# microsoft/PDP-Solver

Measured on AMD Instinct MI355X. Metric: pdp_iterations_per_sec, higher is better.
Workload: dtype f32; 1 GPU; configs[1]: 'p-d-p' survey propagation, random 3-SAT n=200 m=840 batch=5000 T=100 per GPU; E=12600000, V=999999, F=4200000, algorithmic_bytes_per_launch=19540000000, semantics=reference (batch-wide couplings reproduced), parallelism=instances sharded, dp1

## Files before the change

### pdp-solver_amd/csrc/pdp_solve.hip

```cpp
#include "pdp_device.hpp"
#include <stdlib.h>
#include <algorithm>
#include <vector>
#include <type_traits>

#define ST(s) ((hipStream_t)(s))
#define PDP_RETRY_WITH_FORCE (-77)

template <class IT>
struct SView {
    int b, n, m, e;
    const IT *e_var, *e_fn, *v_ptr, *v_edges, *f_ptr, *f_edges;
    const int8_t *sgn;
    float *av, *af, *sol;
    float *emask;
    float *qu; int qstride;
    float *eta; int estride;
    const float *force; int fstride;
    float *s0, *s1, *s2, *s3;
    float *S;
    float *P, *N, *xv1, *xv2, *score, *coeff, *assign;
    int32_t *deg, *sdeg;
    uint8_t *flag_v, *flag_f, *flag_f2;
};
// ... 40 lines not shown
    uint32_t *w_perm_zero, *w_iters_run, *w_violation;
    int team_size, team_count, team_slots;
    int team_no_xcd;
    int exact;
    int rf;
    int isolate;
    uint32_t *risk;
    int no_scorer_reuse;
    int no_event_look;
    int rf_no_fused_step;
    int debug_ghost_inject;
    int adopt_poison;
    int lds_tickets;
    uint8_t *ghost_flag;
    uint32_t *team_ws;
};

struct SolveCtl {
    uint32_t nan_iter;
    uint32_t perm_zero;
    uint32_t violation;
    uint32_t iters_run;
    uint32_t replay_count;
    uint32_t do_replay;
    int32_t poison_from;
    uint32_t ticket;
};
struct SolveCall {
    uint32_t poisoned_all;
    uint32_t stop;
// ... 964 lines not shown
            neg = neg + (negative ? 1.0f : 0.0f) * f;
            all = all + f;
        }
        const float sc = d_score_from_sums(pos, neg, all, ext, pi);
        if (check_score && sc != sc) bad = 1;
    }
    if (bad) cs->found = 1;
    __syncthreads();
    return cs->found;
}

#define DEC_FIXED 1
#define DEC_SPEC_SHIFT 1
#define DEC_VERIFIED_SHIFT 3
template <bool FORCE>
__device__ __noinline__ int lds_decimate(uint32_t smem_off, uint32_t cold_off, int nt, int n, int m, int ne, int cur, int active, float pi, int verified, int scorer_src)
{
    unsigned char *const smem = lds_at<unsigned char>(smem_off);
    ColdShared *const cs = lds_at<ColdShared>(cold_off);
    const LdsArrays L = carve_all(smem, n, m, ne);
    constexpr int VMD = FORCE ? PV_VMASK_RF : 0x3fff;
    const int tid = threadIdx.x, lane = tid & 63;
    float *Enew = cur ? L.EA : L.EB;
    float *score = L.xv2, *assign = L.coeff;
    DEC_PROF_DECL
    float *const SL = (scorer_src == 2) ? L.QU : L.Y;
    const int y_has_logs = scorer_src == 1;
    if (!y_has_logs) {
        const int full = ne / (4 * nt), rem = ne - full * 4 * nt, quarter = (rem + 3) >> 2;
        for (int k = 0; k <= full; ++k) {
            const bool tail = k == full;
// ... 4 lines not shown
            for (int j = 0; j < 4; ++j) { p[j] = p0 + j * st; in[j] = p[j] < ne; if (!in[j]) p[j] = p0; }
            const f4v lg = log4_fin((f4v){1.0f - Enew[p[0]], 1.0f - Enew[p[1]], 1.0f - Enew[p[2]], 1.0f - Enew[p[3]]}, PDP_SCORER_EPS);
            const float r[4] = {lg.x, lg.y, lg.z, lg.w};
#pragma unroll
            for (int j = 0; j < 4; ++j) if (in[j]) SL[p[j]] = r[j] * (0.0f + L.af[L.pcc[p[j]] & 0x3fff]);
        }
    }
    if (tid == 0) { cs->key = 0ull; cs->flags = 0; cs->found = 0; }
    __syncthreads();
    DEC_PROF_MARK(16);
    const float Lpi = pdp_safe_log(1.0f - pi, PDP_SCORER_EPS), L0 = pdp_safe_log(1.0f - pi * 0.0f, PDP_SCORER_EPS);
    const float clamp_sp = y_has_logs ? log2_fin((f2v){0.0f, 0.0f}, PDP_SP_EPS).x : __builtin_nanf(""), clamp_sc = log4_fin((f4v)(0.0f), PDP_SCORER_EPS).x;
    int flags = 0;
    unsigned long long key = 0ull;
    for (int i = tid; i < n; i += nt) {
        const int v = L.vord[i];
        float ext = 0.0f, pos = 0.0f, neg = 0.0f, all = 0.0f;
        auto acc = [&](float f, uint16_t pw, float frc) {
            const bool ng = (pw & 0x8000) != 0;
            f = (f == clamp_sp) ? clamp_sc : f;
            ext = ext + frc;
            pos = pos + (ng ? 0.0f : 1.0f) * f;
            neg = neg + (ng ? 1.0f : 0.0f) * f;
            all = all + f;
        };
        int p = L.v_ptr[v];
        const int bnd = L.v_ptr[v + 1];
        for (; p + 7 < bnd; p += 8) {
            float f[8], fr[8]; uint16_t pw[8];
#pragma unroll
            for (int j = 0; j < 8; ++j) { f[j] = SL[p + j]; pw[j] = L.pvv[p + j]; fr[j] = FORCE ? frc_of(pw[j]) : 0.0f; }
// ... 3 lines not shown
        for (; p + 3 < bnd; p += 4) {
            float f[4], fr[4]; uint16_t pw[4];
#pragma unroll
            for (int j = 0; j < 4; ++j) { f[j] = SL[p + j]; pw[j] = L.pvv[p + j]; fr[j] = FORCE ? frc_of(pw[j]) : 0.0f; }
#pragma unroll
            for (int j = 0; j < 4; ++j) acc(f[j], pw[j], fr[j]);
        }
        for (; p < bnd; ++p) { const uint16_t pw1 = L.pvv[p]; acc(SL[p], pw1, FORCE ? frc_of(pw1) : 0.0f); }
        const float sc = lds_score_of(pos, neg, all, ext, Lpi, L0);
        const float co = (pdp_abs(sc) * L.av[v]) * 1.0f;
        score[v] = sc; L.coeff[v] = co;
        L.flag_v[v] = 0;
        if (co == 0.0f) flags |= 1;
        if (co != 0.0f) flags |= 2;
        if (co != co) flags |= 4;
        const unsigned long long kv = argkey((co - 0.0f) + 1.0f, v);
        key = kv > key ? kv : key;
    }
    flags = wave_reduce(flags, OpOrI(), 0);
    key = wave_max_u64(key);
    if (lane == 63) { if (flags) atomicOr(&cs->flags, flags); if (key) atomicMax(&cs->key, key); }
    __syncthreads();
    flags = UNI(cs->flags);
    const int z3 = flags & 1, anynz = (flags >> 1) & 1, cn = (flags >> 2) & 1;
    int ret = ((z3 ? 1 : 0) | (cn ? 2 : 0)) << DEC_SPEC_SHIFT;
    DEC_PROF_MARK(17);
    const unsigned long long kwin = cs->key;
    const int li = UNI(argkey_index(kwin));
    if (!(active && anynz && !cn && li >= 0)) return ret | (verified << DEC_VERIFIED_SHIFT);
    const float sgn_li = pdp_sign(score[li]);
    DEC_PROF_MARK(18);
    const LView I = make_lview(L, 0, n, m, ne, nt, cs->red, VMD);
    SimplifyScratch ss;
    ss.assign = assign; ss.deg = reinterpret_cast<int32_t *>(L.xv1); ss.sdeg = reinterpret_cast<int32_t *>(L.xv2);
    ss.flag_v = L.flag_v; ss.flag_f = reinterpret_cast<uint8_t *>(L.S); ss.flag_f2 = ss.flag_f + ((m + 15) & ~15); ss.red = cs->red;

    if (verified == 0) {
        int bad = 0;
        for (int c = tid; c < m; c += nt) {
            if (L.af[c] == 1.0f) {
                float deg = 0.0f;
                for (int k = L.f_ptr[c]; k < L.f_ptr[c + 1]; ++k) deg = deg + L.av[L.pvv[L.e2p[k]] & VMD];
                if (deg == 1.0f) bad = 1;
// ... 71 lines not shown
#endif
        if (found & 1) d_simplify(I, ss, &cs->is_sat);
        else if (found & 2) d_peel(I, ss);
        return ret;
    }

    for (int v = tid; v < n; v += nt) assign[v] = 0.0f;
    __syncthreads();
    if (tid == 0) assign[li] = sgn_li;
    __syncthreads();
    d_set_variable_core(I, ss);
    d_simplify(I, ss, &cs->is_sat);
    return ret;
}

__device__ __noinline__ int lds_reinforce_step(uint32_t smem_off, uint32_t cold_off, int nt, int n, int m, int ne, int cur, float pi, int do_force, int logs)
{
    ColdShared *const cs = lds_at<ColdShared>(cold_off);
    const LdsArrays L = carve_all(lds_at<unsigned char>(smem_off), n, m, ne);
    const int tid = threadIdx.x;
    int bad = 0;
    const float *const Enew = cur ? L.EA : L.EB;
    float *const SL = (logs == 2) ? L.QU : L.Y;
    if (do_force && logs != 1) {
        for (int p = tid; p < ne; p += nt)
            SL[p] = pdp_safe_log_fin(1.0f - Enew[p], PDP_SCORER_EPS) * (0.0f + L.af[L.pcc[p] & 0x3fff]);
        __syncthreads();
    }
    const float clamp_sp = (logs == 1) ? pdp_safe_log_fin(0.0f, PDP_SP_EPS) : __builtin_nanf(""), clamp_sc = pdp_safe_log_fin(0.0f, PDP_SCORER_EPS);
    const float Lpi = pdp_safe_log(1.0f - pi, PDP_SCORER_EPS), L0 = pdp_safe_log(1.0f - pi * 0.0f, PDP_SCORER_EPS);
    uint32_t *const codev = reinterpret_cast<uint32_t *>(L.xv2);
    for (int i = tid; i < n; i += nt) {
        const int v = L.vord[i];
        const int a = L.v_ptr[v], bnd = L.v_ptr[v + 1];
        float pred;
        if (do_force) {
            float ext = 0.0f, pos = 0.0f, neg = 0.0f, all = 0.0f;
            const bool in_place = logs == 1 && L.av[v] == 1.0f;
            for (int p = a; p < bnd; ++p) {
                float f = SL[p];
                if (logs == 1) f = in_place ? ((f == clamp_sp) ? clamp_sc : f) : pdp_safe_log_fin(1.0f - Enew[p], PDP_SCORER_EPS) * (0.0f + L.af[L.pcc[p] & 0x3fff]);
                const uint16_t pw = L.pvv[p];
                const bool ng = (pw & 0x8000) != 0;
                ext = ext + frc_of(pw);
                pos = pos + (ng ? 0.0f : 1.0f) * f;
                neg = neg + (ng ? 1.0f : 0.0f) * f;
                all = all + f;
            }
// ... 90 lines not shown
            for (int p = tid; p < ne; p += nt) pvv[p] = (uint16_t)(spv[p] | (frc_enc(sp.frc_in[G.e0 + p]) << PV_FRC_SHIFT));
        }
        asm volatile("s_waitcnt vmcnt(0)" ::: "memory");
    }
    __shared__ __attribute__((aligned(16))) ColdShared s_cold;
    constexpr int SPEC_LOCAL = 64;
    __shared__ uint8_t s_spec_used[SPEC_LOCAL], s_spec_zero[SPEC_LOCAL];
    __shared__ int s_flag_or[2];
    __shared__ int s_sat_count;
    __shared__ uint32_t s_risk;
    __shared__ int s_poison;
    if (tid < SPEC_LOCAL) { s_spec_used[tid] = 0; s_spec_zero[tid] = 0; }
    if (tid == 0) { s_cold.is_sat = hdr.is_sat; s_flag_or[0] = 0; s_flag_or[1] = 0; s_sat_count = 0; s_risk = 0xffffffffu; }
    __syncthreads();

    const bool p4_cached = 2 * n <= nt;
    uint32_t p4_lohi = 0u, p4_vdeg = 0u;
    if (p4_cached && tid < 2 * n) {
        const int v = L.vord[tid >> 1], h = tid & 1;
        const int a = L.v_ptr[v], bnd = L.v_ptr[v + 1];
        const int half = (bnd - a + 1) >> 1;
        p4_lohi = (uint32_t)(a + h * half) | ((uint32_t)(h ? bnd : a + half) << 16);
        p4_vdeg = (uint32_t)v | ((uint32_t)(bnd - a) << 16);
    }
    int active = hdr.active ? 1 : 0;
    int has_prev = sp.has_prev;
    int last_event = -1;
    int prev_from_global = (sp.has_prev && sp.prev_slots) ? 1 : 0;
    int use_em = sp.has_edge_mask, last_use_em = 0, em_dirty = 0;
    float cnt = hdr.cnt;
    int iters = 0, did_prop = 0, violation = 0, cur = 0;
    int logs_ready = 0;
    int qu_is_delta = 0;
    int mask_fix = 0;
// ... 51 lines not shown
                if (((c >> 1) ^ c) & PC_EM_USED) pcc[p] = (uint16_t)((c & ~PC_EM_USED) | ((c & PC_EM) ? PC_EM_USED : 0));
            }
            __syncthreads();
            PROF_MARK(19);
        }
        last_use_em = use_em; em_dirty = 0; mask_fix = 0;
        PROF_MARK(1);
        {
            const uint16_t *const e2p = L.e2p, *const f_ptr = L.f_ptr, *const v_ptr = L.v_ptr;
            float *const S = L.S;
            const int nvi = (n + 63) >> 6, nci = (m + 63) >> 6;
            const uint16_t *const vord = L.vord;
            auto var_rows = [&](int item) {
                const int i = (item << 6) + lane;
                if (i >= n) return;
                const int v = vord[i];
                float P = 0.0f, N = 0.0f;
                const int a = v_ptr[v], bnd = v_ptr[v + 1];
                auto acc = [&](float y, uint16_t sg) {
                    const uint32_t neg = (uint32_t)((int32_t)((uint32_t)sg << 16) >> 31);
                    P = P + __uint_as_float(__float_as_uint(y) & ~neg);
                    N = N + __uint_as_float(__float_as_uint(y) & neg);
                };
                int p = a;
                for (; p + 15 < bnd; p += 16) {
                    float y[16]; uint16_t sg[16];
#pragma unroll
                    for (int j = 0; j < 16; ++j) { y[j] = Y[p + j]; sg[j] = pvv[p + j]; }
#pragma unroll
                    for (int j = 0; j < 16; ++j) acc(y[j], sg[j]);
                }
// ... 153 lines not shown
        qu_is_delta = logs_ready;
        float *const Dsrc = fuse_logs ? QU : Y;
        __syncthreads();
        PROF_MARK(3);
        int bits = nan_seen ? 4 : 0;
        {
            const uint16_t *const v_ptr = L.v_ptr;
            const float *const av = L.av;
            float *const amb = L.xv1;
            const float tol_lo = tol - (2e-6f + 1e-4f * pdp_abs(tol)), tol_hi = tol + (2e-6f + 1e-4f * pdp_abs(tol));
            if (!PROF_SKIP(8))
            for (int r = tid; r < 2 * n; r += nt) {
                int v, lo, hi, degi;
                if (p4_cached) { lo = (int)(p4_lohi & 0xffffu); hi = (int)(p4_lohi >> 16); v = (int)(p4_vdeg & 0xffffu); degi = (int)(p4_vdeg >> 16); }
                else {
                    v = L.vord[r >> 1];
                    const int h = r & 1, a = v_ptr[v], bnd = v_ptr[v + 1];
                    const int half = (bnd - a + 1) >> 1;
                    lo = a + h * half; hi = h ? bnd : a + half; degi = bnd - a;
                }
                float emax = 0.0f, S1 = 0.0f, S2 = 0.0f, D = 0.0f;
                if (has_prev) {
                    int p = lo;
                    for (; p + 1 < hi; p += 2) {
                        const float e0 = Enew[p], e1 = Enew[p + 1], d0 = Dsrc[p], d1 = Dsrc[p + 1];
                        emax = fmaxf(emax, fmaxf(e0, e1));
                        S1 += d0 + d1; S2 = fmaf(d0, d0, fmaf(d1, d1, S2)); D = fmaxf(D, fmaxf(d0, d1));
                    }
                    if (p < hi) { const float e0 = Enew[p], d0 = Dsrc[p]; emax = fmaxf(emax, e0); S1 += d0; S2 = fmaf(d0, d0, S2); D = fmaxf(D, d0); }
                } else {
                    for (int p = lo; p < hi; ++p) emax = fmaxf(emax, Enew[p]);
// ... 104 lines not shown
                conv = below_tol ? 1 : 0;
                if (cnt >= t_max) { conv = 1; cnt = 0.0f; }
                if (conv) last_event = t;
            }
        } else if (has_prev) {
            if (cnt >= t_max) { conv = 1; cnt = 0.0f; }
        }
        uint32_t used = (RF ? 0u : 1u) | (has_prev ? 2u : 0u);
        uint32_t zero = ((!RF && z1) ? 1u : 0u) | ((has_prev && z2) ? 2u : 0u);
        if (!RF && has_prev && !conv && n > 0) zero |= 4u;
        if constexpr (RF) {
            const int flip = (sp.coins[sp.chunk_start + t] < sp.dprob) && active;
            rf_last_flip = flip;
            if (flip || nsat < 0) {
                const int keep_logs = fuse_logs ? (use_em ? 1 : 2) : 0;
                if (UNI(lds_reinforce_step(lds_offset_of(smem), lds_offset_of(&s_cold), nt, n, m, ne, cur, pi, flip, keep_logs)) && !nan_seen) violation = 1;
                rf_changed = 1;
                if (!keep_logs) logs_ready = 0;
            }
        }
        PROF_MARK(13);
        int decimated = 0;
        if (!RF && has_prev && conv && !poisoned && !nan_seen && !PROF_SKIP(16)) {
            const int scorer_src = !fuse_logs ? 0 : ((use_em && !sp.no_scorer_reuse) ? 1 : 2);
            const int dr = UNI(lds_decimate<FORCE>(lds_offset_of(smem), lds_offset_of(&s_cold), nt, n, m, ne, cur, active, pi, simplified, scorer_src));
            decimated = dr & DEC_FIXED; simplified = (dr >> DEC_VERIFIED_SHIFT) & 3;
            const int spec_bits = (dr >> DEC_SPEC_SHIFT) & 3;
            used |= 4u;
            if (spec_bits & 1) zero |= 4u;
            if (spec_bits & 2) violation = 1;
        }
        if (decimated) { if (simplified == 1) PROF_COUNT(10); else PROF_COUNT(11); }
        PROF_COUNT(12);
        PROF_MARK(6);
        if (has_prev) cnt = cnt + 1.0f;
        if (tid == 0 && !poisoned) {
            if (t < SPEC_LOCAL) { s_spec_used[t] = (uint8_t)used; s_spec_zero[t] = (uint8_t)zero; }
            else { atomicOr(&sp.spec_used[t], used); if (zero) atomicOr(&sp.spec_zero[t], zero); }
        }
        {
// ... 50 lines not shown
            if (sp.check_termination && active && nsat == m) active = 0;
        }
        has_prev = 1; prev_from_global = 0; cur ^= 1;
        PROF_MARK(15);
    }

    int any_inactive = 0;
    for (int v = tid; v < n; v += nt) any_inactive |= (L.av[v] == 0.0f) ? 1 : 0;
    any_inactive = __syncthreads_or(any_inactive);
    const bool finishing = did_prop && (sp.final_chunk || !active);
    float *const Efin = cur ? L.EB : L.EA, *const Eprev = cur ? L.EA : L.EB;
    const bool ghost = finishing && !active && !(sp.final_chunk && iters >= T) && !sp.isolate;
    if (finishing) {
        float *gq = sp.q + 3 * (size_t)G.e0;
        float *gfs = sp.fs + 2 * (size_t)G.e0;
        for (int p = tid; p < ne; p += nt) {
            const int e = G.v_edges[p];
            const uint16_t pw = pvv[p], cw = pcc[p];
            const int v = pw & VM;
            const float s = slot_sign(pw);
            float y = pdp_safe_log_fin(1.0f - Eprev[p], PDP_SP_EPS);
            if (last_use_em) y = y * ((cw & PC_EM_USED) ? 1.0f : 0.0f);
            const float force = RF ? (rf_last_flip ? (qu_is_delta ? QU[p] : X[p]) : frc_of(pw)) : (FORCE ? frc_of(pw) : 0.0f);
            const float pos = 0.0f + L.PN[2 * v], neg = 0.0f + L.PN[2 * v + 1];
            float same = (0.5f * (1.0f + s)) * pos + (0.5f * (1.0f - s)) * neg;
            same = same - y;
            same = same + ((force == s) ? L1 : L0);
            float opp = (0.5f * (1.0f - s)) * pos + (0.5f * (1.0f + s)) * neg;
            opp = opp + ((force == -s) ? L1 : L0);
            const float dc = pdp_expf_fin_le30(same + opp);
            const float A = pdp_expf_fin_le30(same), Bv = pdp_expf_fin_le30(opp);
            const float qu = A * (1.0f - Bv), qs = Bv * (1.0f - A);
            const float total = (qu + qs) + dc;
            const float sticky = qu_is_delta ? __builtin_fmaf(1.0f - 1.0f, X[p], qu / total) : QU[p];
            const float sticky_out = (ghost && sp.debug_ghost_inject && p == 0) ? __builtin_nanf("") : sticky;
            if (ghost) QU[p] = sticky_out;
            gq[3 * e] = sticky_out;
            gq[3 * e + 1] = 1.0f * (qs / total) + (1.0f - 1.0f) * sticky;
            gq[3 * e + 2] = 1.0f * (dc / total) + (1.0f - 1.0f) * sticky;
            gfs[2 * e] = Efin[p];
            if constexpr (RF) gfs[2 * e + 1] = frc_of(pw);
            sp.prev[G.e0 + e] = Efin[p];
            G.emask[e] = (cw & PC_EM) ? 1.0f : 0.0f;
        }
        for (int v = tid; v < n; v += nt) { G.av[v] = L.av[v]; G.sol[v] = L.sol[v]; }
        for (int c = tid; c < m; c += nt) G.af[c] = L.af[c];
    } else {
        auto dump16 = [&](size_t off, const void *src, size_t bytes) {
            uint4 *g = reinterpret_cast<uint4 *>(dout + off);
            const uint4 *d = reinterpret_cast<const uint4 *>(src);
            for (int i = tid; i < (int)((bytes + 15) >> 4); i += nt) g[i] = d[i];
        };
        dump16(BL.QU, QU, (size_t)ne * 4); dump16(BL.E, Efin, (size_t)ne * 4);
        dump16(BL.af, L.af, (size_t)m * 4); dump16(BL.av, L.av, (size_t)n * 4); dump16(BL.sol, L.sol, (size_t)n * 4);
        uint16_t *gpc = reinterpret_cast<uint16_t *>(dout + BL.pcc);
        for (int p = tid; p < ne; p += nt) { const uint16_t cw = pcc[p]; gpc[p] = (uint16_t)((cw & ~PC_EM_USED) | ((cw & PC_EM) ? PC_EM_USED : 0)); }
        if constexpr (RF) { for (int p = tid; p < ne; p += nt) sp.frc_out[G.e0 + p] = frc_of(pvv[p]); }
    }
    int ghost_bad = 0;
    if (ghost) {
// ... 19 lines not shown
        if (!REPLAY) sp.last_event[gb] = last_event;
        if (sp.risk) sp.risk[gb] = finishing ? 0xffffffffu : s_risk;
        atomicMax(&ctl->iters_run, (uint32_t)iters);
        if (violation) atomicOr(&ctl->violation, 1u);
    }
}

struct SolveSnapshot {
    float *q, *fs, *av, *af, *sol, *sat, *emask, *prev, *cnt; uint8_t *amask;
};
__global__ void __launch_bounds__(256) k_solve_import(PView pv, const float *q, const float *fs, const uint8_t *amask, const float *prev, const float *counters,
                                                      int has_prev, int build_static, char *stat, char *dyn, const int64_t *stat_off, const int64_t *dyn_off, float *prev_slots,
                                                      const int32_t *list, int stage_cap ,
                                                      SolveCall *force_check ,
                                                      int use_em ,
                                                      SolveSnapshot snap )
{
    const Inst G = load_inst(pv, list ? list[blockIdx.x] : (int)blockIdx.x);
    const int n = G.n, m = G.m, ne = G.e, tid = threadIdx.x, nt = blockDim.x;
    const BlobLayout BL = blob_layout(n, m, ne);
    char *st = stat + stat_off[G.b], *dy = dyn + dyn_off[G.b];
    uint16_t *pvv = reinterpret_cast<uint16_t *>(st + BL.pvv), *e2p = reinterpret_cast<uint16_t *>(st + BL.e2p);
    float *QU = reinterpret_cast<float *>(dy + BL.QU), *Ecur = reinterpret_cast<float *>(dy + BL.E);
    uint16_t *pcc = reinterpret_cast<uint16_t *>(dy + BL.pcc);
    const float *sq = q + 3 * (size_t)G.e0, *sfs = fs + 2 * (size_t)G.e0;
    extern __shared__ __attribute__((aligned(16))) float stage[];
    if (force_check) {
        int some = 0;
        for (int e0 = tid; e0 < ne; e0 += 4 * nt) {
            float f[4];
#pragma unroll
            for (int j = 0; j < 4; ++j) { const int e = e0 + j * nt; f[j] = sfs[2 * (e < ne ? e : e0) + 1]; }
#pragma unroll
            for (int j = 0; j < 4; ++j) some |= (f[j] != 0.0f) ? 1 : 0;
        }
        if (__syncthreads_or(some) && tid == 0) atomicOr(&force_check->force_seen, 1u);
    }
// ... 7 lines not shown
                const int e = (e0 + j * nt < ne) ? e0 + j * nt : e0;
                qv[j] = sq[3 * e]; ev[j] = sfs[2 * e]; fn[j] = G.e_fn[e];
                if (use_em) mv[j] = G.emask[e];
                if (has_prev) pv[j] = prev[G.e0 + e];
            }
#pragma unroll
            for (int j = 0; j < 4; ++j) {
                const int e = e0 + j * nt;
                if (e >= ne) continue;
                sQ[e] = qv[j]; sE[e] = ev[j]; sC[e] = (uint16_t)(fn[j] | ((mv[j] == 1.0f) ? (PC_EM | PC_EM_USED) : 0));
                if (has_prev) sP[e] = pv[j];
            }
        }
        __syncthreads();
        for (int p0 = tid; p0 < ne; p0 += 8 * nt) {
            int e[8], evar[8], esg[8];
#pragma unroll
            for (int j = 0; j < 8; ++j) { const int p = p0 + j * nt; e[j] = G.v_edges[p < ne ? p : p0]; }
            if (build_static) {
#pragma unroll
                for (int j = 0; j < 8; ++j) { evar[j] = G.e_var[e[j]]; esg[j] = G.sgn[e[j]]; }
            }
#pragma unroll
            for (int j = 0; j < 8; ++j) {
                const int p = p0 + j * nt;
                if (p >= ne) continue;
                if (build_static) { pvv[p] = (uint16_t)(evar[j] | (esg[j] < 0 ? 0x8000 : 0)); e2p[e[j]] = (uint16_t)p; }
                pcc[p] = sC[e[j]];
                QU[p] = sQ[e[j]]; Ecur[p] = sE[e[j]];
                if (has_prev) prev_slots[G.e0 + p] = sP[e[j]];
            }
        }
    } else
    for (int p0 = tid; p0 < ne; p0 += 4 * nt) {
        int e[4]; float qv[4], ev[4], mv[4], pv[4] = {0.0f, 0.0f, 0.0f, 0.0f}; int fn[4];
#pragma unroll
        for (int j = 0; j < 4; ++j) { const int p = p0 + j * nt; e[j] = G.v_edges[p < ne ? p : p0]; }
#pragma unroll
        for (int j = 0; j < 4; ++j) {
            qv[j] = sq[3 * e[j]]; ev[j] = sfs[2 * e[j]]; mv[j] = use_em ? G.emask[e[j]] : 1.0f; fn[j] = G.e_fn[e[j]];
            if (has_prev) pv[j] = prev[G.e0 + e[j]];
        }
#pragma unroll
        for (int j = 0; j < 4; ++j) {
            const int p = p0 + j * nt;
            if (p >= ne) continue;
            if (build_static) { pvv[p] = (uint16_t)(G.e_var[e[j]] | (G.sgn[e[j]] < 0 ? 0x8000 : 0)); e2p[e[j]] = (uint16_t)p; }
            pcc[p] = (uint16_t)(fn[j] | ((mv[j] == 1.0f) ? (PC_EM | PC_EM_USED) : 0));
            QU[p] = qv[j]; Ecur[p] = ev[j];
            if (has_prev) prev_slots[G.e0 + p] = pv[j];
        }
    }
    if (build_static) {
        uint16_t *vp = reinterpret_cast<uint16_t *>(st + BL.vptr), *fp = reinterpret_cast<uint16_t *>(st + BL.fptr);
        for (int v = tid; v <= n; v += nt) vp[v] = (uint16_t)G.v_ptr[v];
        for (int c = tid; c <= m; c += nt) fp[c] = (uint16_t)G.f_ptr[c];
        __shared__ int hist[256];
        uint16_t *vord = reinterpret_cast<uint16_t *>(st + BL.vord);
        for (int i = tid; i < 256; i += nt) hist[i] = 0;
        __syncthreads();
        for (int v = tid; v < n; v += nt) { const int d = G.v_ptr[v + 1] - G.v_ptr[v]; atomicAdd(&hist[255 - (d < 255 ? d : 255)], 1); }
        __syncthreads();
        if (tid == 0) { int run = 0; for (int i = 0; i < 256; ++i) { const int c = hist[i]; hist[i] = run; run += c; } }
        __syncthreads();
        for (int v = tid; v < n; v += nt) { const int d = G.v_ptr[v + 1] - G.v_ptr[v]; vord[atomicAdd(&hist[255 - (d < 255 ? d : 255)], 1)] = (uint16_t)v; }
    }
    float *av = reinterpret_cast<float *>(dy + BL.av), *sol = reinterpret_cast<float *>(dy + BL.sol), *af = reinterpret_cast<float *>(dy + BL.af);
    int any_inactive = 0;
    for (int v = tid; v < n; v += nt) {
        const float a = G.av[v], so = G.sol[v];
        av[v] = a; sol[v] = so; any_inactive |= (a == 0.0f) ? 1 : 0;
        if (snap.av) { snap.av[G.v0 + v] = a; snap.sol[G.v0 + v] = so; }
    }
    for (int c = tid; c < m; c += nt) { const float f = G.af[c]; af[c] = f; if (snap.av) snap.af[G.f0 + c] = f; }
    any_inactive = __syncthreads_or(any_inactive);
    if (tid == 0) {
        if (snap.av) { snap.sat[G.b] = pv.is_sat[G.b]; snap.cnt[G.b] = counters[G.b]; snap.amask[G.b] = amask[G.b]; }
        DynHeader h;
        h.active = amask[G.b] ? 1u : 0u; h.done = h.active ? 0u : 1u;
        h.perm_zero = (h.done && any_inactive) ? 1u : 0u; h.simplified = 0;
        h.cnt = counters[G.b]; h.is_sat = pv.is_sat[G.b]; h.nsat_p1 = 0; h.pad2 = 0.0f;
        *reinterpret_cast<DynHeader *>(dy + BL.hdr) = h;
    }
}

__global__ void __launch_bounds__(256) k_force_import(PView pv, const float *fs, float *frc, SolveCtl *ctl0, const uint8_t *amask)
{
    const Inst G = load_inst(pv, blockIdx.x);
    if (!amask[G.b]) return;
    const float *sfs = fs + 2 * (size_t)G.e0;
    int odd = 0;
    for (int p = threadIdx.x; p < G.e; p += blockDim.x) {
        const float f = sfs[2 * G.v_edges[p] + 1];
        frc[G.e0 + p] = f;
        odd |= (f == f && f != 0.0f && f != 1.0f && f != -1.0f) ? 1 : 0;
    }
    if (__syncthreads_or(odd) && threadIdx.x == 0) atomicOr(&ctl0->violation, 1u);
}

__global__ void __launch_bounds__(1024) k_solve_post(SolveCtl *ctl, SolveCall *call, int c, int isolate, int B, const int32_t *last_event, int32_t *list,
                                                     const uint8_t *is_big)
{
    __shared__ int s_from;
    if (threadIdx.x == 0) {
        int from = -1;
        if (!call->stop) {
            ctl->do_replay = 0; ctl->replay_count = 0;
            if (!isolate && !call->poisoned_all && ctl->nan_iter < (uint32_t)c) {
// ... 279 lines not shown
        if (!instance_fits_lds(n, m, e)) { big.push_back((int32_t)b); is_big[b] = 1; continue; }
        fit.push_back((int32_t)b);
        if (n > p->res_fit_n) p->res_fit_n = n;
        if (m > p->res_fit_m) p->res_fit_m = m;
        if (e > p->res_fit_e) p->res_fit_e = e;
        const BlobLayout bl = blob_layout(n, m, e);
        so += bl.stat_bytes; dy += bl.dyn_bytes;
    }
    p->res_nfit = (int)fit.size(); p->res_nbig = (int)big.size();
    { int st_ = pdp_dev_alloc((void **)&p->res_fit_list, (fit.size() + 1) * 4); if (st_ != PDP_OK) return st_; }
    { int st_ = pdp_dev_alloc((void **)&p->res_big_list, (big.size() + 1) * 4); if (st_ != PDP_OK) return st_; }
    { int st_ = pdp_dev_alloc((void **)&p->res_is_big, B + 1); if (st_ != PDP_OK) return st_; }
    if (!fit.empty()) PDP_HIP_CHECK(hipMemcpy(p->res_fit_list, fit.data(), fit.size() * 4, hipMemcpyHostToDevice));
    if (!big.empty()) PDP_HIP_CHECK(hipMemcpy(p->res_big_list, big.data(), big.size() * 4, hipMemcpyHostToDevice));
    PDP_HIP_CHECK(hipMemcpy(p->res_is_big, is_big.data(), B, hipMemcpyHostToDevice));
    p->res_stat_bytes = so + 16; p->res_dyn_bytes = dy + 16;
    { int st_ = pdp_dev_alloc((void **)&p->res_stat, p->res_stat_bytes); if (st_ != PDP_OK) return st_; }
    { int st_ = pdp_dev_alloc((void **)&p->res_dyn[0], p->res_dyn_bytes); if (st_ != PDP_OK) return st_; }
    { int st_ = pdp_dev_alloc((void **)&p->res_dyn[1], p->res_dyn_bytes); if (st_ != PDP_OK) return st_; }
    { int st_ = pdp_dev_alloc((void **)&p->res_prev_slots, (E + 4) * sizeof(float)); if (st_ != PDP_OK) return st_; }
    p->res_static_built = 0;
    { int st_ = pdp_dev_alloc((void **)&p->res_stat_off, 2 * B * sizeof(int64_t)); if (st_ != PDP_OK) return st_; }
    PDP_HIP_CHECK(hipMemcpy(p->res_stat_off, off.data(), 2 * B * sizeof(int64_t), hipMemcpyHostToDevice));
    return PDP_OK;
}

static int hbm_workspaces(pdp_problem *p, SolveParams &sp, bool records = true)
{
    for (int i = 0; i < 4; ++i) sp.ws_e[i] = p->ws_e[i];
    sp.ws_f = p->ws_f[0];
    for (int i = 0; i < 6; ++i) sp.ws_v[i] = p->ws_v[i];
    if (!p->solve_extra_v) { int st_ = pdp_dev_alloc((void **)&p->solve_extra_v, sizeof(float) * (size_t)p->V); if (st_ != PDP_OK) return st_; }
    sp.ws_v[6] = p->solve_extra_v;
    for (int i = 0; i < 3; ++i) sp.ws_vi[i] = p->ws_vi[i];
    sp.ws_fu[0] = p->ws_fu[0]; sp.ws_fu[1] = p->ws_fu[1];
    if (records) {
        if (!p->solve_rec) { int st_ = pdp_dev_alloc((void **)&p->solve_rec, sizeof(float) * 4 * ((size_t)p->E + 4)); if (st_ != PDP_OK) return st_; }
        sp.ws_r = p->solve_rec;
    }
    return PDP_OK;
// ... 78 lines not shown
    int32_t *order = (int32_t *)(risk + B + 8);
    int ticket_extra = nbig > 0 ? 25 : 0;
    if (const char *env = getenv("PDP_SOLVE_TICKETS")) ticket_extra = atoi(env);
    const bool risk_order = nbig == 0 && ticket_extra <= 0 && !fit_list && nchunks > 1 && !a->isolate_instances && getenv("PDP_SOLVE_NO_RISK_ORDER") == nullptr;
    {
        const int words = 2 * T, cover = (int)B > words ? (int)B : words;
        hipLaunchKernelGGL(k_solve_ctl_init, dim3(((cover > nchunks ? cover : nchunks) + 255) / 256), dim3(256), 0, st, ctl, nchunks, call, spec, words, ghost_flag, (int)B,
                           risk_order ? order : (int32_t *)nullptr, risk);
    }
    int stage_cap = (p->res_fit_e + 7) & ~7;
    const size_t stage_per_edge = a->decimator->has_prev ? 14 : 10;
    if ((size_t)stage_cap * stage_per_edge > 159 * 1024) stage_cap = 0;
    if (getenv("PDP_SOLVE_IMPORT_GATHER")) stage_cap = 0;
    const size_t stage_bytes = (size_t)stage_cap * stage_per_edge;
    if (stage_bytes > 64 * 1024) PDP_HIP_CHECK(hipFuncSetAttribute((const void *)k_solve_import, hipFuncAttributeMaxDynamicSharedMemorySize, (int)stage_bytes));
    hipLaunchKernelGGL(k_solve_import, dim3(nfit), dim3(256), stage_bytes, st, make_view(p), (const float *)a->q, (const float *)a->fs, (const uint8_t *)a->active_mask,
                       (const float *)a->decimator->prev, (const float *)a->decimator->counters, a->decimator->has_prev, p->res_static_built ? 0 : 1,
                       p->res_stat, p->res_dyn[0], stat_off, dyn_off, p->res_prev_slots, fit_list, stage_cap, (force || rf) ? (SolveCall *)nullptr : call,
                       p->has_edge_mask ? 1 : 0, snap_in_import ? snap0 : SolveSnapshot{});
    PDP_LAUNCH_CHECK();
    p->res_static_built = 1;

    SolveParams sp;
    memset(&sp, 0, sizeof(sp));
    sp.tol = a->tolerance; sp.t_max = a->t_max; sp.pi = a->pi;
    sp.q = a->q; sp.fs = a->fs; sp.amask = a->active_mask; sp.src_fs = a->fs;
    sp.prev = a->decimator->prev; sp.counters = a->decimator->counters;
    sp.check_termination = a->check_termination;
    sp.coins = a->coins; sp.dprob = a->decimation_probability;
    sp.rf = rf ? 1 : 0; sp.isolate = a->isolate_instances ? 1 : 0;
    sp.adopt_poison = getenv("PDP_SOLVE_NO_ADOPT") ? 0 : 1;
    sp.debug_ghost_inject = getenv("PDP_DEBUG_GHOST_INJECT") ? 1 : 0;
    sp.no_scorer_reuse = getenv("PDP_SOLVE_NO_SCORER_REUSE") ? 1 : 0;
    sp.no_event_look = getenv("PDP_SOLVE_NO_EVENT_LOOK") ? 1 : 0;
    sp.rf_no_fused_step = getenv("PDP_SOLVE_RF_NO_FUSED_STEP") ? 1 : 0;
    if (rf || force) {
        hipLaunchKernelGGL(k_force_import, dim3(p->B), dim3(256), 0, st, make_view(p), (const float *)a->fs, frc_buf[0], ctl, (const uint8_t *)a->active_mask);
    }
    sp.ghost_flag = ghost_flag;
    sp.last_event = last_event; sp.inst_list = replay_list;
    sp.call = call; sp.stat = p->res_stat; sp.stat_off = stat_off; sp.dyn_off = dyn_off;
    sp.fit_list = fit_list;
    BigSnap big_live, big_snap;
    if (nbig) {
        { const int st_ = hbm_workspaces(p, sp); if (st_ != PDP_OK) return st_; }
        sp.big_list = p->res_big_list; sp.hbm_device_ctl = 1;
        status = ensure_bytes(&p->res_big_snap, &p->res_big_snap_bytes, snap_bytes + 64);
        if (status != PDP_OK) return status;
        float *f = (float *)p->res_big_snap;
        big_snap.q = f; f += 3 * E; big_snap.fs = f; f += 2 * E; big_snap.av = f; f += V; big_snap.af = f; f += F; big_snap.sol = f; f += V;
        big_snap.sat = f; f += B; big_snap.emask = f; f += E; big_snap.prev = f; f += E; big_snap.cnt = f; f += B; big_snap.amask = (uint8_t *)f;
        big_live.q = a->q; big_live.fs = a->fs; big_live.av = p->av; big_live.af = p->af; big_live.sol = p->sol; big_live.sat = p->is_sat;
        big_live.emask = p->emask; big_live.prev = a->decimator->prev; big_live.cnt = a->decimator->counters; big_live.amask = a->active_mask;
// ... 443 lines not shown
```

Before: 12380 iterations/s (each iteration sweeps a batch of 5000 instances).

## Renumber variables in degree-sorted order inside resident LDS layout

Builds the per-instance static layout so that variable slots and edge slots are laid out in descending-degree order (vord), with a stored slot-to-edge map, instead of natural variable order with an indirection through vord. Kernel loops then index variables directly by position, and results are scattered back to caller variable ids at export, with argmax keys carrying both the caller and the local index so tie-breaking is preserved. This is meant to remove the vord indirection and give contiguous, load-balanced edge runs per wave. The cost is extra static-build work and an added slot_edge buffer, and the renumbering could break tie-breaking or other paths that assume natural ids. An env var restores natural order.

```diff
diff --git a/pdp-solver_amd/csrc/pdp_solve.hip b/pdp-solver_amd/csrc/pdp_solve.hip
--- a/pdp-solver_amd/csrc/pdp_solve.hip
+++ b/pdp-solver_amd/csrc/pdp_solve.hip
@@ -78,6 +78,7 @@
     int lds_tickets;
     uint8_t *ghost_flag;
     uint32_t *team_ws;
+    int natural_order;
 };
 
 struct SolveCtl {
@@ -1072,7 +1073,7 @@
 #define DEC_SPEC_SHIFT 1
 #define DEC_VERIFIED_SHIFT 3
 template <bool FORCE>
-__device__ __noinline__ int lds_decimate(uint32_t smem_off, uint32_t cold_off, int nt, int n, int m, int ne, int cur, int active, float pi, int verified, int scorer_src)
+__device__ __noinline__ int lds_decimate(uint32_t smem_off, uint32_t cold_off, int nt, int n, int m, int ne, int cur, int active, float pi, int verified, int scorer_src, int nat)
 {
     unsigned char *const smem = lds_at<unsigned char>(smem_off);
     ColdShared *const cs = lds_at<ColdShared>(cold_off);
@@ -1107,7 +1108,9 @@
     int flags = 0;
     unsigned long long key = 0ull;
     for (int i = tid; i < n; i += nt) {
-        const int v = L.vord[i];
+        const int w = L.vord[i];
+        const int v = nat ? w : i;
+        const int v_caller = nat ? v : w;
         float ext = 0.0f, pos = 0.0f, neg = 0.0f, all = 0.0f;
         auto acc = [&](float f, uint16_t pw, float frc) {
             const bool ng = (pw & 0x8000) != 0;
@@ -1141,7 +1144,7 @@
         if (co == 0.0f) flags |= 1;
         if (co != 0.0f) flags |= 2;
         if (co != co) flags |= 4;
-        const unsigned long long kv = argkey((co - 0.0f) + 1.0f, v);
+        const unsigned long long kv = argkey((co - 0.0f) + 1.0f, (v_caller << 16) | v);
         key = kv > key ? kv : key;
     }
     flags = wave_reduce(flags, OpOrI(), 0);
@@ -1153,7 +1156,8 @@
     int ret = ((z3 ? 1 : 0) | (cn ? 2 : 0)) << DEC_SPEC_SHIFT;
     DEC_PROF_MARK(17);
     const unsigned long long kwin = cs->key;
-    const int li = UNI(argkey_index(kwin));
+    const int li_pair = UNI(argkey_index(kwin));
+    const int li = li_pair < 0 ? -1 : (li_pair & 0xffff);
     if (!(active && anynz && !cn && li >= 0)) return ret | (verified << DEC_VERIFIED_SHIFT);
     const float sgn_li = pdp_sign(score[li]);
     DEC_PROF_MARK(18);
@@ -1255,7 +1259,7 @@
     return ret;
 }
 
-__device__ __noinline__ int lds_reinforce_step(uint32_t smem_off, uint32_t cold_off, int nt, int n, int m, int ne, int cur, float pi, int do_force, int logs)
+__device__ __noinline__ int lds_reinforce_step(uint32_t smem_off, uint32_t cold_off, int nt, int n, int m, int ne, int cur, float pi, int do_force, int logs, int nat)
 {
     ColdShared *const cs = lds_at<ColdShared>(cold_off);
     const LdsArrays L = carve_all(lds_at<unsigned char>(smem_off), n, m, ne);
@@ -1272,7 +1276,7 @@
     const float Lpi = pdp_safe_log(1.0f - pi, PDP_SCORER_EPS), L0 = pdp_safe_log(1.0f - pi * 0.0f, PDP_SCORER_EPS);
     uint32_t *const codev = reinterpret_cast<uint32_t *>(L.xv2);
     for (int i = tid; i < n; i += nt) {
-        const int v = L.vord[i];
+        const int v = nat ? (int)L.vord[i] : i;
         const int a = L.v_ptr[v], bnd = L.v_ptr[v + 1];
         float pred;
         if (do_force) {
@@ -1393,10 +1397,11 @@
     if (tid == 0) { s_cold.is_sat = hdr.is_sat; s_flag_or[0] = 0; s_flag_or[1] = 0; s_sat_count = 0; s_risk = 0xffffffffu; }
     __syncthreads();
 
+    const bool nat = sp.natural_order != 0;
     const bool p4_cached = 2 * n <= nt;
     uint32_t p4_lohi = 0u, p4_vdeg = 0u;
     if (p4_cached && tid < 2 * n) {
-        const int v = L.vord[tid >> 1], h = tid & 1;
+        const int v = nat ? (int)L.vord[tid >> 1] : (tid >> 1), h = tid & 1;
         const int a = L.v_ptr[v], bnd = L.v_ptr[v + 1];
         const int half = (bnd - a + 1) >> 1;
         p4_lohi = (uint32_t)(a + h * half) | ((uint32_t)(h ? bnd : a + half) << 16);
@@ -1478,7 +1483,7 @@
             auto var_rows = [&](int item) {
                 const int i = (item << 6) + lane;
                 if (i >= n) return;
-                const int v = vord[i];
+                const int v = nat ? (int)vord[i] : i;
                 float P = 0.0f, N = 0.0f;
                 const int a = v_ptr[v], bnd = v_ptr[v + 1];
                 auto acc = [&](float y, uint16_t sg) {
@@ -1662,7 +1667,7 @@
                 int v, lo, hi, degi;
                 if (p4_cached) { lo = (int)(p4_lohi & 0xffffu); hi = (int)(p4_lohi >> 16); v = (int)(p4_vdeg & 0xffffu); degi = (int)(p4_vdeg >> 16); }
                 else {
-                    v = L.vord[r >> 1];
+                    v = nat ? (int)L.vord[r >> 1] : (r >> 1);
                     const int h = r & 1, a = v_ptr[v], bnd = v_ptr[v + 1];
                     const int half = (bnd - a + 1) >> 1;
                     lo = a + h * half; hi = h ? bnd : a + half; degi = bnd - a;
@@ -1797,7 +1802,7 @@
             rf_last_flip = flip;
             if (flip || nsat < 0) {
                 const int keep_logs = fuse_logs ? (use_em ? 1 : 2) : 0;
-                if (UNI(lds_reinforce_step(lds_offset_of(smem), lds_offset_of(&s_cold), nt, n, m, ne, cur, pi, flip, keep_logs)) && !nan_seen) violation = 1;
+                if (UNI(lds_reinforce_step(lds_offset_of(smem), lds_offset_of(&s_cold), nt, n, m, ne, cur, pi, flip, keep_logs, nat ? 1 : 0)) && !nan_seen) violation = 1;
                 rf_changed = 1;
                 if (!keep_logs) logs_ready = 0;
             }
@@ -1806,7 +1811,7 @@
         int decimated = 0;
         if (!RF && has_prev && conv && !poisoned && !nan_seen && !PROF_SKIP(16)) {
             const int scorer_src = !fuse_logs ? 0 : ((use_em && !sp.no_scorer_reuse) ? 1 : 2);
-            const int dr = UNI(lds_decimate<FORCE>(lds_offset_of(smem), lds_offset_of(&s_cold), nt, n, m, ne, cur, active, pi, simplified, scorer_src));
+            const int dr = UNI(lds_decimate<FORCE>(lds_offset_of(smem), lds_offset_of(&s_cold), nt, n, m, ne, cur, active, pi, simplified, scorer_src, nat ? 1 : 0));
             decimated = dr & DEC_FIXED; simplified = (dr >> DEC_VERIFIED_SHIFT) & 3;
             const int spec_bits = (dr >> DEC_SPEC_SHIFT) & 3;
             used |= 4u;
@@ -1887,8 +1892,8 @@
     if (finishing) {
         float *gq = sp.q + 3 * (size_t)G.e0;
         float *gfs = sp.fs + 2 * (size_t)G.e0;
-        for (int p = tid; p < ne; p += nt) {
-            const int e = G.v_edges[p];
+        for (int e = tid; e < ne; e += nt) {
+            const int p = L.e2p[e];
             const uint16_t pw = pvv[p], cw = pcc[p];
             const int v = pw & VM;
             const float s = slot_sign(pw);
@@ -1916,7 +1921,7 @@
             sp.prev[G.e0 + e] = Efin[p];
             G.emask[e] = (cw & PC_EM) ? 1.0f : 0.0f;
         }
-        for (int v = tid; v < n; v += nt) { G.av[v] = L.av[v]; G.sol[v] = L.sol[v]; }
+        for (int v = tid; v < n; v += nt) { const int vc = nat ? v : (int)L.vord[v]; G.av[vc] = L.av[v]; G.sol[vc] = L.sol[v]; }
         for (int c = tid; c < m; c += nt) G.af[c] = L.af[c];
     } else {
         auto dump16 = [&](size_t off, const void *src, size_t bytes) {
@@ -1966,13 +1971,56 @@
                                                       const int32_t *list, int stage_cap ,
                                                       SolveCall *force_check ,
                                                       int use_em ,
-                                                      SolveSnapshot snap )
+                                                      SolveSnapshot snap ,
+                                                      int natural ,
+                                                      uint16_t *slot_edge )
 {
     const Inst G = load_inst(pv, list ? list[blockIdx.x] : (int)blockIdx.x);
     const int n = G.n, m = G.m, ne = G.e, tid = threadIdx.x, nt = blockDim.x;
     const BlobLayout BL = blob_layout(n, m, ne);
     char *st = stat + stat_off[G.b], *dy = dyn + dyn_off[G.b];
     uint16_t *pvv = reinterpret_cast<uint16_t *>(st + BL.pvv), *e2p = reinterpret_cast<uint16_t *>(st + BL.e2p);
+    uint16_t *const vord = reinterpret_cast<uint16_t *>(st + BL.vord), *const sedge = slot_edge + G.e0;
+    if (build_static) {
+        __shared__ int hist[256];
+        uint16_t *vp = reinterpret_cast<uint16_t *>(st + BL.vptr), *fp = reinterpret_cast<uint16_t *>(st + BL.fptr);
+        for (int i = tid; i < 256; i += nt) hist[i] = 0;
+        __syncthreads();
+        for (int v = tid; v < n; v += nt) { const int d = G.v_ptr[v + 1] - G.v_ptr[v]; atomicAdd(&hist[255 - (d < 255 ? d : 255)], 1); }
+        __syncthreads();
+        if (tid == 0) { int run = 0; for (int i = 0; i < 256; ++i) { const int c = hist[i]; hist[i] = run; run += c; } }
+        __syncthreads();
+        for (int v = tid; v < n; v += nt) { const int d = G.v_ptr[v + 1] - G.v_ptr[v]; vord[atomicAdd(&hist[255 - (d < 255 ? d : 255)], 1)] = (uint16_t)v; }
+        __syncthreads();
+        if (natural) {
+            for (int v = tid; v <= n; v += nt) vp[v] = (uint16_t)G.v_ptr[v];
+        } else {
+            const int run_len = (n + nt - 1) / nt, i0 = min(n, tid * run_len), i1 = min(n, i0 + run_len);
+            int sum = 0;
+            for (int i = i0; i < i1; ++i) { const int v = vord[i]; sum += G.v_ptr[v + 1] - G.v_ptr[v]; }
+            for (int t = tid; t < 256; t += nt) hist[t] = 0;
+            __syncthreads();
+            if (tid < 256) hist[tid] = sum;
+            __syncthreads();
+            if (tid == 0) { int run = 0; for (int t = 0; t < 256; ++t) { const int c = hist[t]; hist[t] = run; run += c; } }
+            __syncthreads();
+            int at = hist[tid < 256 ? tid : 255];
+            for (int i = i0; i < i1; ++i) { const int v = vord[i]; vp[i] = (uint16_t)at; at += G.v_ptr[v + 1] - G.v_ptr[v]; }
+            if (tid == 0) vp[n] = (uint16_t)ne;
+        }
+        for (int c = tid; c <= m; c += nt) fp[c] = (uint16_t)G.f_ptr[c];
+        __syncthreads();
+        for (int i = tid; i < n; i += nt) {
+            const int v = natural ? i : (int)vord[i];
+            const int a = G.v_ptr[v], d = G.v_ptr[v + 1] - a, base = vp[i];
+            for (int j = 0; j < d; ++j) {
+                const int e = G.v_edges[a + j], p = base + j;
+                sedge[p] = (uint16_t)e; e2p[e] = (uint16_t)p;
+                pvv[p] = (uint16_t)(i | (G.sgn[e] < 0 ? 0x8000 : 0));
+            }
+        }
+        __syncthreads();
+    }
     float *QU = reinterpret_cast<float *>(dy + BL.QU), *Ecur = reinterpret_cast<float *>(dy + BL.E);
     uint16_t *pcc = reinterpret_cast<uint16_t *>(dy + BL.pcc);
     const float *sq = q + 3 * (size_t)G.e0, *sfs = fs + 2 * (size_t)G.e0;
@@ -2010,18 +2058,13 @@
         }
         __syncthreads();
         for (int p0 = tid; p0 < ne; p0 += 8 * nt) {
-            int e[8], evar[8], esg[8];
-#pragma unroll
-            for (int j = 0; j < 8; ++j) { const int p = p0 + j * nt; e[j] = G.v_edges[p < ne ? p : p0]; }
-            if (build_static) {
-#pragma unroll
-                for (int j = 0; j < 8; ++j) { evar[j] = G.e_var[e[j]]; esg[j] = G.sgn[e[j]]; }
-            }
+            int e[8];
+#pragma unroll
+            for (int j = 0; j < 8; ++j) { const int p = p0 + j * nt; e[j] = sedge[p < ne ? p : p0]; }
 #pragma unroll
             for (int j = 0; j < 8; ++j) {
                 const int p = p0 + j * nt;
                 if (p >= ne) continue;
-                if (build_static) { pvv[p] = (uint16_t)(evar[j] | (esg[j] < 0 ? 0x8000 : 0)); e2p[e[j]] = (uint16_t)p; }
                 pcc[p] = sC[e[j]];
                 QU[p] = sQ[e[j]]; Ecur[p] = sE[e[j]];
                 if (has_prev) prev_slots[G.e0 + p] = sP[e[j]];
@@ -2031,7 +2074,7 @@
     for (int p0 = tid; p0 < ne; p0 += 4 * nt) {
         int e[4]; float qv[4], ev[4], mv[4], pv[4] = {0.0f, 0.0f, 0.0f, 0.0f}; int fn[4];
 #pragma unroll
-        for (int j = 0; j < 4; ++j) { const int p = p0 + j * nt; e[j] = G.v_edges[p < ne ? p : p0]; }
+        for (int j = 0; j < 4; ++j) { const int p = p0 + j * nt; e[j] = sedge[p < ne ? p : p0]; }
 #pragma unroll
         for (int j = 0; j < 4; ++j) {
             qv[j] = sq[3 * e[j]]; ev[j] = sfs[2 * e[j]]; mv[j] = use_em ? G.emask[e[j]] : 1.0f; fn[j] = G.e_fn[e[j]];
@@ -2041,31 +2084,17 @@
         for (int j = 0; j < 4; ++j) {
             const int p = p0 + j * nt;
             if (p >= ne) continue;
-            if (build_static) { pvv[p] = (uint16_t)(G.e_var[e[j]] | (G.sgn[e[j]] < 0 ? 0x8000 : 0)); e2p[e[j]] = (uint16_t)p; }
             pcc[p] = (uint16_t)(fn[j] | ((mv[j] == 1.0f) ? (PC_EM | PC_EM_USED) : 0));
             QU[p] = qv[j]; Ecur[p] = ev[j];
             if (has_prev) prev_slots[G.e0 + p] = pv[j];
         }
     }
-    if (build_static) {
-        uint16_t *vp = reinterpret_cast<uint16_t *>(st + BL.vptr), *fp = reinterpret_cast<uint16_t *>(st + BL.fptr);
-        for (int v = tid; v <= n; v += nt) vp[v] = (uint16_t)G.v_ptr[v];
-        for (int c = tid; c <= m; c += nt) fp[c] = (uint16_t)G.f_ptr[c];
-        __shared__ int hist[256];
-        uint16_t *vord = reinterpret_cast<uint16_t *>(st + BL.vord);
-        for (int i = tid; i < 256; i += nt) hist[i] = 0;
-        __syncthreads();
-        for (int v = tid; v < n; v += nt) { const int d = G.v_ptr[v + 1] - G.v_ptr[v]; atomicAdd(&hist[255 - (d < 255 ? d : 255)], 1); }
-        __syncthreads();
-        if (tid == 0) { int run = 0; for (int i = 0; i < 256; ++i) { const int c = hist[i]; hist[i] = run; run += c; } }
-        __syncthreads();
-        for (int v = tid; v < n; v += nt) { const int d = G.v_ptr[v + 1] - G.v_ptr[v]; vord[atomicAdd(&hist[255 - (d < 255 ? d : 255)], 1)] = (uint16_t)v; }
-    }
     float *av = reinterpret_cast<float *>(dy + BL.av), *sol = reinterpret_cast<float *>(dy + BL.sol), *af = reinterpret_cast<float *>(dy + BL.af);
     int any_inactive = 0;
-    for (int v = tid; v < n; v += nt) {
+    for (int i = tid; i < n; i += nt) {
+        const int v = natural ? i : (int)vord[i];
         const float a = G.av[v], so = G.sol[v];
-        av[v] = a; sol[v] = so; any_inactive |= (a == 0.0f) ? 1 : 0;
+        av[i] = a; sol[i] = so; any_inactive |= (a == 0.0f) ? 1 : 0;
         if (snap.av) { snap.av[G.v0 + v] = a; snap.sol[G.v0 + v] = so; }
     }
     for (int c = tid; c < m; c += nt) { const float f = G.af[c]; af[c] = f; if (snap.av) snap.af[G.f0 + c] = f; }
@@ -2080,14 +2109,17 @@
     }
 }
 
-__global__ void __launch_bounds__(256) k_force_import(PView pv, const float *fs, float *frc, SolveCtl *ctl0, const uint8_t *amask)
+__global__ void __launch_bounds__(256) k_force_import(PView pv, const float *fs, float *frc, SolveCtl *ctl0, const uint8_t *amask, const uint16_t *slot_edge,
+                                                      const uint8_t *is_big)
 {
     const Inst G = load_inst(pv, blockIdx.x);
     if (!amask[G.b]) return;
+    const bool big = is_big[G.b] != 0;
     const float *sfs = fs + 2 * (size_t)G.e0;
+    const uint16_t *const sedge = slot_edge + G.e0;
     int odd = 0;
     for (int p = threadIdx.x; p < G.e; p += blockDim.x) {
-        const float f = sfs[2 * G.v_edges[p] + 1];
+        const float f = sfs[2 * (big ? G.v_edges[p] : (int)sedge[p]) + 1];
         frc[G.e0 + p] = f;
         odd |= (f == f && f != 0.0f && f != 1.0f && f != -1.0f) ? 1 : 0;
     }
@@ -2397,7 +2429,7 @@
     if (!fit.empty()) PDP_HIP_CHECK(hipMemcpy(p->res_fit_list, fit.data(), fit.size() * 4, hipMemcpyHostToDevice));
     if (!big.empty()) PDP_HIP_CHECK(hipMemcpy(p->res_big_list, big.data(), big.size() * 4, hipMemcpyHostToDevice));
     PDP_HIP_CHECK(hipMemcpy(p->res_is_big, is_big.data(), B, hipMemcpyHostToDevice));
-    p->res_stat_bytes = so + 16; p->res_dyn_bytes = dy + 16;
+    p->res_stat_bytes = ((so + 16 + 15) & ~(size_t)15) + 2 * (E + 8); p->res_dyn_bytes = dy + 16;
     { int st_ = pdp_dev_alloc((void **)&p->res_stat, p->res_stat_bytes); if (st_ != PDP_OK) return st_; }
     { int st_ = pdp_dev_alloc((void **)&p->res_dyn[0], p->res_dyn_bytes); if (st_ != PDP_OK) return st_; }
     { int st_ = pdp_dev_alloc((void **)&p->res_dyn[1], p->res_dyn_bytes); if (st_ != PDP_OK) return st_; }
@@ -2407,6 +2439,8 @@
     PDP_HIP_CHECK(hipMemcpy(p->res_stat_off, off.data(), 2 * B * sizeof(int64_t), hipMemcpyHostToDevice));
     return PDP_OK;
 }
+
+static uint16_t *resident_slot_edge(const pdp_problem *p) { return reinterpret_cast<uint16_t *>(p->res_stat + p->res_stat_bytes - 2 * ((size_t)p->E + 8)); }
 
 static int hbm_workspaces(pdp_problem *p, SolveParams &sp, bool records = true)
 {
@@ -2515,12 +2549,14 @@
     if (getenv("PDP_SOLVE_IMPORT_GATHER")) stage_cap = 0;
     const size_t stage_bytes = (size_t)stage_cap * stage_per_edge;
     if (stage_bytes > 64 * 1024) PDP_HIP_CHECK(hipFuncSetAttribute((const void *)k_solve_import, hipFuncAttributeMaxDynamicSharedMemorySize, (int)stage_bytes));
+    const int build_static = p->res_static_built ? 0 : 1;
+    const int natural = build_static ? (getenv("PDP_SOLVE_NATURAL_VAR_ORDER") ? 1 : 0) : (p->res_static_built == 2 ? 1 : 0);
     hipLaunchKernelGGL(k_solve_import, dim3(nfit), dim3(256), stage_bytes, st, make_view(p), (const float *)a->q, (const float *)a->fs, (const uint8_t *)a->active_mask,
-                       (const float *)a->decimator->prev, (const float *)a->decimator->counters, a->decimator->has_prev, p->res_static_built ? 0 : 1,
+                       (const float *)a->decimator->prev, (const float *)a->decimator->counters, a->decimator->has_prev, build_static,
                        p->res_stat, p->res_dyn[0], stat_off, dyn_off, p->res_prev_slots, fit_list, stage_cap, (force || rf) ? (SolveCall *)nullptr : call,
-                       p->has_edge_mask ? 1 : 0, snap_in_import ? snap0 : SolveSnapshot{});
+                       p->has_edge_mask ? 1 : 0, snap_in_import ? snap0 : SolveSnapshot{}, natural, resident_slot_edge(p));
     PDP_LAUNCH_CHECK();
-    p->res_static_built = 1;
+    p->res_static_built = natural ? 2 : 1;
 
     SolveParams sp;
     memset(&sp, 0, sizeof(sp));
@@ -2536,8 +2572,10 @@
     sp.no_event_look = getenv("PDP_SOLVE_NO_EVENT_LOOK") ? 1 : 0;
     sp.rf_no_fused_step = getenv("PDP_SOLVE_RF_NO_FUSED_STEP") ? 1 : 0;
     if (rf || force) {
-        hipLaunchKernelGGL(k_force_import, dim3(p->B), dim3(256), 0, st, make_view(p), (const float *)a->fs, frc_buf[0], ctl, (const uint8_t *)a->active_mask);
-    }
+        hipLaunchKernelGGL(k_force_import, dim3(p->B), dim3(256), 0, st, make_view(p), (const float *)a->fs, frc_buf[0], ctl, (const uint8_t *)a->active_mask,
+                           (const uint16_t *)resident_slot_edge(p), (const uint8_t *)p->res_is_big);
+    }
+    sp.natural_order = natural;
     sp.ghost_flag = ghost_flag;
     sp.last_event = last_event; sp.inst_list = replay_list;
     sp.call = call; sp.stat = p->res_stat; sp.stat_off = stat_off; sp.dyn_off = dyn_off;
```

Result: no change. 12450 iterations/s (each iteration sweeps a batch of 5000 instances), median of 6 (+0.6%).
